# mjmyt/drone_path_planning_python

Measured on AMD Instinct MI355X. Metric: minimum-snap trajectories/sec (N drones × M segments, order 7) at 1/2/4/8 MI355X, higher is better.
Workload: dtype f64

## Files before the change

drone_path_planning_python_amd/csrc/msnap_aux.hip:

```cpp
#include <math.h>

#include <cstdlib>

#include "msnap_internal.h"
#include "msnap_energy.h"

namespace msnap {

__global__ void __launch_bounds__(256)
pack_kernel(const double *__restrict__ coef, const double *__restrict__ dur, float *__restrict__ out,
            size_t n_rows , int nc) {
  const int ncol = 1 + 4 * nc;
  const size_t total = n_rows * (size_t)ncol;
  for (size_t idx = (size_t)blockIdx.x * blockDim.x + threadIdx.x; idx < total;
       idx += (size_t)gridDim.x * blockDim.x) {
    const size_t row = idx / ncol;
    const int col = (int)(idx - row * ncol);
    const double v = (col == 0) ? dur[row] : coef[row * (size_t)(4 * nc) + (col - 1)];
    out[idx] = (float)v;
  }
}

int launch_pack(msnap_ctx *ctx, int n_drones, int n_seg, const double *coef, const double *dur, float *out) {
  const size_t rows = (size_t)n_drones * n_seg;
// ... 196 lines not shown
  const bool aligned = ((size_t)d0 * per_drone & 1) == 0;
  if (aligned) {
    for (size_t e = (size_t)tid * 2; e + 1 < words; e += (size_t)nthreads * 2)
      *reinterpret_cast<double2 *>(out + e) = *reinterpret_cast<const double2 *>(sImg + e);
    if ((words & 1) && tid == 0) out[words - 1] = sImg[words - 1];
  } else {
    for (size_t e = tid; e < words; e += nthreads) out[e] = sImg[e];
  }
  if (pos_t != nullptr) {
    const int runs = (int)per_drone;
    for (int e = tid; e < runs * nd; e += nthreads) {
      const int sk = e / nd, dl = e - sk * nd;
      pos_t[(size_t)sk * Rp + d0 + dl] = sImg[(size_t)dl * per_drone + sk];
    }
  }
  if (kbox != nullptr) {
    const int dl = tid >> 4, part = tid & 15;
    double lo[3] = {INFINITY, INFINITY, INFINITY}, hi[3] = {-INFINITY, -INFINITY, -INFINITY};
    if (dl < nd) {
      const double *img = sImg + (size_t)dl * per_drone;
      for (int sq = part; sq < S; sq += 16)
#pragma unroll
        for (int k = 0; k < 3; ++k) {
          const double v = img[(size_t)sq * 3 + k];
          if (__builtin_isfinite(v)) {
            lo[k] = v < lo[k] ? v : lo[k];
            hi[k] = v > hi[k] ? v : hi[k];
          }
        }
    }
#pragma unroll
    for (int m = 1; m < 16; m <<= 1)
#pragma unroll
      for (int k = 0; k < 3; ++k) {
        const double ol = shfl_xor_f64(lo[k], m), oh = shfl_xor_f64(hi[k], m);
        lo[k] = ol < lo[k] ? ol : lo[k];
        hi[k] = oh > hi[k] ? oh : hi[k];
      }
    if (dl < nd && part == 0) {
      double *b = kbox + (size_t)(d0 + dl) * 6;
#pragma unroll
      for (int k = 0; k < 3; ++k) {
        b[k] = lo[k];
        b[3 + k] = hi[k];
      }
      kkey[d0 + dl] = drone_sort_key(lo, hi);
    }
  }
}

__device__ __forceinline__ unsigned div_magic(unsigned d) { return d > 1 ? 0xffffffffu / d + 1u : 0u; }
__device__ __forceinline__ int div_by(int x, unsigned magic) { return magic ? (int)__umulhi((unsigned)x, magic) : x; }

template <int NC>
__global__ void __launch_bounds__(256)
sample_kernel(const double *__restrict__ coef, const double *__restrict__ dur, double dt, int N, int M, int S,
              int naxes, int DW, double *__restrict__ pos, double *__restrict__ pos_t, int Rp, double *__restrict__ kbox,
              unsigned *__restrict__ kkey) {
#pragma clang fp contract(off)
  extern __shared__ __attribute__((aligned(16))) double smem[];
  double *sB = smem;
  int *sGen = reinterpret_cast<int *>(sB + (size_t)DW * (M + 1));
  double *sImg = reinterpret_cast<double *>(sGen + ((DW + 1) & ~1));
  const int tid = threadIdx.x;
  const size_t per_drone = (size_t)S * naxes;
  const unsigned inv_piece = div_magic((unsigned)(naxes * M)), inv_axes = div_magic((unsigned)naxes);
  for (int d0 = blockIdx.x * DW; d0 < N; d0 += gridDim.x * DW) {
    const int nd = N - d0 < DW ? N - d0 : DW;
    if (tid < nd) {
      const double *dr = dur + (size_t)(d0 + tid) * M;
      double acc = 0.0;
      bool ranges = dt > 0.0;
      sB[tid * (M + 1)] = 0.0;
      for (int i = 0; i < M; ++i) {
        const double Ti = dr[i];
        ranges = ranges && (Ti >= 0.0);
        acc = acc + Ti;
        sB[tid * (M + 1) + i + 1] = acc;
      }
      sGen[tid] = ranges ? 0 : 1;
    }
    __syncthreads();
    const int items = nd * M * naxes;
    for (int it = tid; it < items; it += blockDim.x) {
      const int dl = div_by(it, inv_piece), rem = it - dl * (naxes * M);
      const int i = div_by(rem, inv_axes), a = rem - i * naxes;
      const double *cbase = coef + (size_t)(d0 + dl) * M * 4 * NC;
      double *img = sImg + (size_t)dl * per_drone;
      if (sGen[dl]) {
        if (i == 0)
          for (int sq = 0; sq < S; ++sq)
            sample_point_generic<NC>(cbase, dur + (size_t)(d0 + dl) * M, M, (double)sq * dt, a, img[(size_t)sq * naxes + a]);
        continue;
      }
      const double *crow = cbase + ((size_t)i * 4 + a) * NC;
      sample_piece<NC>(sB[dl * (M + 1) + i], sB[dl * (M + 1) + i + 1], i, M, S, dt, img, naxes, a, [&](double (&c)[NC]) {
#pragma unroll
        for (int q = 0; q < NC; q += 2) {
          const double2 v = *reinterpret_cast<const double2 *>(crow + q);
          c[q] = v.x;
          c[q + 1] = v.y;
        }
      });
    }
    __syncthreads();
    sample_image_out(sImg, tid, blockDim.x, nd, d0, per_drone, S, pos, pos_t, Rp, kbox, kkey);
    __syncthreads();
  }
}

#ifdef MSNAP_TOOLS_TIMELINE
__device__ unsigned long long g_gs_timeline[1024 * 8];
#define MSNAP_GSTL(k)                                              \
  do {                                                             \
    if (threadIdx.x == 0) s_gs_tl[(k)] = wall_clock64();           \
  } while (0)
#define MSNAP_GSTL_FLUSH()                                                                   \
  do {                                                                                       \
    lds_barrier();                                                                           \
    if (threadIdx.x < 8 && blockIdx.x < 1024) g_gs_timeline[blockIdx.x * 8 + threadIdx.x] = s_gs_tl[threadIdx.x]; \
  } while (0)
}
extern "C" int msnap_debug_read_gs_timeline(unsigned long long *out, int n_words) {
  if (hipDeviceSynchronize() != hipSuccess) return MSNAP_EHIP;
  return hipMemcpyFromSymbol(out, HIP_SYMBOL(msnap::g_gs_timeline), (size_t)n_words * 8) == hipSuccess ? MSNAP_OK : MSNAP_EHIP;
}
namespace msnap {
#else
#define MSNAP_GSTL(k) do { } while (0)
#define MSNAP_GSTL_FLUSH() do { } while (0)
#endif

typedef double v4f64s __attribute__((ext_vector_type(4)));
constexpr int kFuseKS = 3;
constexpr int kFuseTasks = 4;

template <int NC>
__global__ void __launch_bounds__(256, 2)
grid_sample_kernel(const double *__restrict__ wp, const double *__restrict__ frag, int ks_pitch,
                   const double *__restrict__ gdur, const int32_t *__restrict__ gstatus, double dt, int N, int M, int S,
                   int DW, double *__restrict__ coef, double *__restrict__ dur, int32_t *__restrict__ status,
                   double *__restrict__ pos, double *__restrict__ pos_t, int Rp, double *__restrict__ kbox,
                   unsigned *__restrict__ kkey) {
#pragma clang fp contract(off)
  extern __shared__ __attribute__((aligned(16))) double smem[];
  const int m = M + 1, ncols = M * NC, nct = (ncols + 15) >> 4, nks = (m + 3) >> 2;
  const int nrt = (DW * 4 + 15) >> 4, rows16 = nrt * 16, ntasks = nrt * nct;
  const int wpitch = m | 1, cpitch = ncols + 2;
  const int nrt_inv = nrt == 3 ? 86 : 256 >> (nrt >> 1);
  const unsigned m4_inv = (1u << 20) / (unsigned)(m * 4) + 1u;
  const unsigned inv_piece = div_magic((unsigned)(3 * M));
  double *sB = smem;
  double *sW = sB + ((m + 1) & ~1);
  double *sC = sW + (((size_t)rows16 * wpitch + 1) & ~(size_t)1);
  double *sImg = sC + (size_t)DW * 4 * cpitch;
  int *sBad = reinterpret_cast<int *>(sImg + (size_t)DW * S * 3);
  const int tid = threadIdx.x, lane = tid & (kWave - 1);
  const int wave = __builtin_amdgcn_readfirstlane(tid >> 6);
  const int col = lane & 15, kq = lane >> 4;
  const int grid_st = gstatus[0];
  const size_t per_drone = (size_t)S * 3;
#ifdef MSNAP_TOOLS_TIMELINE
  __shared__ unsigned long long s_gs_tl[8];
#endif
  MSNAP_GSTL(0);

  if (tid == 0) {
    double acc = 0.0;
    bool ranges = dt > 0.0;
    sB[0] = 0.0;
    for (int i = 0; i < M; ++i) {
      const double Ti = gdur[i];
      ranges = ranges && (Ti >= 0.0);
      acc = acc + Ti;
      sB[i + 1] = acc;
    }
    sBad[DW] = ranges ? 0 : 1;
  }
  for (int e = tid; e < rows16 * wpitch; e += blockDim.x) sW[e] = 0.0;

  for (int d0 = blockIdx.x * DW; d0 < N; d0 += gridDim.x * DW) {
    const int nd = N - d0 < DW ? N - d0 : DW;
    const int words = nd * m * 4;
    const double *wsrc = wp + (size_t)d0 * m * 4;
    const int e0 = tid, e1 = tid + 256;
    const double w0 = wsrc[e0 < words ? e0 : 0], w1 = wsrc[e1 < words ? e1 : 0];
    double bq[kFuseTasks][kFuseKS];
#pragma unroll
    for (int ti = 0; ti < kFuseTasks; ++ti) {
      const int t = wave + 4 * ti < ntasks ? wave + 4 * ti : ntasks - 1;
      const double *bsrc = frag + (size_t)((t * nrt_inv) >> 8) * ks_pitch * kWave + lane;
#pragma unroll
      for (int ks = 0; ks < kFuseKS; ++ks) bq[ti][ks] = bsrc[(ks < nks ? ks : 0) * kWave];
    }
    if (tid < DW) sBad[tid] = 0;
    lds_barrier();
    MSNAP_GSTL(1);
#pragma unroll
    for (int h = 0; h < 2; ++h) {
      const int e = h ? e1 : e0;
      const double w = h ? w1 : w0;
      if (e < words) {
        const int dl = (int)(((unsigned)e * m4_inv) >> 20), r = e - dl * (m * 4);
        sW[(size_t)(dl * 4 + (r & 3)) * wpitch + (r >> 2)] = w;
        if (!__builtin_isfinite(w)) sBad[dl] = 1;
      }
    }
    lds_barrier();
    MSNAP_GSTL(2);
    {
      double av[kFuseTasks][kFuseKS];
#pragma unroll
      for (int ti = 0; ti < kFuseTasks; ++ti) {
        const int t = wave + 4 * ti < ntasks ? wave + 4 * ti : ntasks - 1;
        const double *arow = sW + (size_t)((t - ((t * nrt_inv) >> 8) * nrt) * 16 + col) * wpitch;
#pragma unroll
        for (int ks = 0; ks < kFuseKS; ++ks) {
          const int j = 4 * ks + kq;
          const double v = arow[j < m ? j : m - 1];
          av[ti][ks] = j < m ? v : 0.0;
        }
      }
      v4f64s acc[kFuseTasks];
#pragma unroll
      for (int ti = 0; ti < kFuseTasks; ++ti) acc[ti] = v4f64s{0.0, 0.0, 0.0, 0.0};
#pragma unroll
      for (int ks = 0; ks < kFuseKS; ++ks)
        if (ks < nks) {
#pragma unroll
          for (int ti = 0; ti < kFuseTasks; ++ti)
            acc[ti] = __builtin_amdgcn_mfma_f64_16x16x4f64(av[ti][ks], bq[ti][ks], acc[ti], 0, 0, 0);
        }
#pragma unroll
      for (int ti = 0; ti < kFuseTasks; ++ti) {
        const int t = wave + 4 * ti;
        const int ct = (t * nrt_inv) >> 8, rt = t - ct * nrt;
        const int c = 16 * ct + col;
        if (t < ntasks && c < ncols) {
#pragma unroll
          for (int r = 0; r < 4; ++r) {
            const int dl = rt * 4 + r;
            if (dl < DW) sC[(size_t)(dl * 4 + kq) * cpitch + c] = acc[ti][r];
          }
        }
      }
    }
    MSNAP_GSTL(7);
    lds_barrier();
    MSNAP_GSTL(3);
    {
      const int ppd = M * 4 * NC / 2;
      for (int dl = wave; dl < nd; dl += 4) {
        const bool bad = grid_st != 0 || sBad[dl] != 0;
        double *cout = coef + (size_t)(d0 + dl) * M * 4 * NC;
        for (int e = lane; e < ppd; e += kWave) {
          const int g = 2 * e;
          const int kc = g % NC, q = g / NC;
          const int a = q & 3, seg = q >> 2;
          double2 v = *reinterpret_cast<const double2 *>(sC + (size_t)(dl * 4 + a) * cpitch + seg * NC + kc);
          if (bad) v = make_double2(__builtin_nan(""), __builtin_nan(""));
          *reinterpret_cast<double2 *>(cout + g) = v;
        }
      }
      for (int e = tid; e < nd * M; e += blockDim.x) dur[(size_t)d0 * M + e] = gdur[e % M];
      if (tid < nd) status[d0 + tid] = sBad[tid] ? MSNAP_ST_NONFINITE : grid_st;
    }
    MSNAP_GSTL(4);
    const int items = nd * M * 3;
    const bool generic = sBad[DW] != 0;
    for (int it = tid; it < items; it += blockDim.x) {
      const int dl = div_by(it, inv_piece), rem = it - dl * (3 * M);
      const int i = rem / 3, a = rem - i * 3;
      double *img = sImg + (size_t)dl * per_drone;
      const double *cbase = sC + (size_t)dl * 4 * cpitch;
      const bool bad = grid_st != 0 || sBad[dl] != 0;
      if (generic || bad) {
        if (i == 0)
          for (int sq = 0; sq < S; ++sq) {
            double x = __builtin_nan("");
            if (!bad) sample_point_generic<NC>(cbase, gdur, M, (double)sq * dt, a, x, NC, cpitch);
            img[(size_t)sq * 3 + a] = x;
          }
        continue;
      }
      const double *crow = cbase + (size_t)a * cpitch + i * NC;
      sample_piece<NC>(sB[i], sB[i + 1], i, M, S, dt, img, 3, a, [&](double (&c)[NC]) {
#pragma unroll
        for (int q = 0; q < NC; q += 2) {
          const double2 v = *reinterpret_cast<const double2 *>(crow + q);
          c[q] = v.x;
          c[q + 1] = v.y;
        }
      });
    }
    lds_barrier();
    MSNAP_GSTL(5);
    sample_image_out(sImg, tid, blockDim.x, nd, d0, per_drone, S, pos, pos_t, Rp, kbox, kkey);
    lds_barrier();
    MSNAP_GSTL(6);
  }
  MSNAP_GSTL_FLUSH();
}

__global__ void collide_key_kernel(const double *__restrict__ pos, int N, int S, double *__restrict__ box,
                                   unsigned *__restrict__ key);
constexpr int kKeyDrones = 4;

int launch_sample(msnap_ctx *ctx, int n_drones, int n_seg, const double *coef, const double *dur, double dt,
                  int n_samples, int n_axes, double *pos, double *pos_t, bool keys_form) {
  const int Rp = (n_drones + kRowBlockRows - 1) / kRowBlockRows * kRowBlockRows;
  double *kbox = keys_form ? pos_t : nullptr;
  unsigned *kkey = keys_form ? reinterpret_cast<unsigned *>(pos_t + (size_t)n_drones * 6) : nullptr;
  if (keys_form) pos_t = nullptr;
  const size_t img_per_drone = (size_t)n_samples * n_axes * sizeof(double);
  int dw = 256 / (n_seg * n_axes);
  if (dw < 1) dw = 1;
  if (dw > 16) dw = 16;
  while (dw > 1 && dw * img_per_drone > 48 * 1024) --dw;
  const size_t lds = ((size_t)dw * (n_seg + 1)) * sizeof(double) + (((size_t)dw + 1) & ~(size_t)1) * sizeof(int) +
                     dw * img_per_drone;
  if (lds <= 64 * 1024) {
    size_t blocks = ((size_t)n_drones + dw - 1) / dw;
    if (blocks > (size_t)ctx->n_cu * 64) blocks = (size_t)ctx->n_cu * 64;
    if (ctx->order == 7)
      hipLaunchKernelGGL((sample_kernel<8>), dim3((unsigned)blocks), dim3(256), lds, ctx->stream, coef, dur, dt,
                         n_drones, n_seg, n_samples, n_axes, dw, pos, pos_t, Rp, kbox, kkey);
    else
      hipLaunchKernelGGL((sample_kernel<10>), dim3((unsigned)blocks), dim3(256), lds, ctx->stream, coef, dur, dt,
                         n_drones, n_seg, n_samples, n_axes, dw, pos, pos_t, Rp, kbox, kkey);
  } else {
    const size_t total = (size_t)n_drones * n_samples;
    size_t blocks = (total + 255) / 256;
    if (blocks > (size_t)ctx->n_cu * 16) blocks = (size_t)ctx->n_cu * 16;
    if (ctx->order == 7)
      hipLaunchKernelGGL((sample_generic_kernel<8>), dim3((unsigned)blocks), dim3(256), 0, ctx->stream, coef, dur, dt,
                         n_drones, n_seg, n_samples, n_axes, pos);
    else
      hipLaunchKernelGGL((sample_generic_kernel<10>), dim3((unsigned)blocks), dim3(256), 0, ctx->stream, coef, dur, dt,
                         n_drones, n_seg, n_samples, n_axes, pos);
    if (pos_t != nullptr) {
      MSNAP_HIP(ctx, hipGetLastError());
      const int E = n_samples * 3;
      hipLaunchKernelGGL(collide_transpose_kernel, dim3(Rp / 64, (E + 31) / 32), dim3(256), 0, ctx->stream,
                         (const double *)pos, n_drones, Rp, E, pos_t, (E + 31) / 32, (int32_t *)nullptr, (size_t)0,
                         (const int32_t *)nullptr, (double *)nullptr);
    }
    if (kbox != nullptr) {
      MSNAP_HIP(ctx, hipGetLastError());
      hipLaunchKernelGGL(collide_key_kernel, dim3((n_drones + kKeyDrones - 1) / kKeyDrones), dim3(kWave * kKeyDrones), 0,
                         ctx->stream, (const double *)pos, n_drones, n_samples, kbox, kkey);
    }
  }
  MSNAP_HIP(ctx, hipGetLastError());
  return MSNAP_OK;
}

int launch_grid_sample(msnap_ctx *ctx, int n_drones, const double *wp, double dt, int n_samples, double *coef,
                       double *dur, int32_t *status, double *pos, double *pos_t, bool keys_form) {
  const int M = ctx->grid_seg, m = M + 1, nc = ctx->order + 1;
  const int ks_pitch = grid_frag_ks_pitch(ctx, M);
  const size_t img_per_drone = (size_t)n_samples * 3 * sizeof(double);
  const int ncols = M * nc, nct = (ncols + 15) / 16, nks = (m + 3) / 4;
  int dw = 256 / (M * 3);
  if (dw > 16) dw = 16;
  auto lds_of = [&](int d) -> size_t {
    const size_t rows16 = (size_t)((d * 4 + 15) / 16) * 16;
    return (size_t)(((m + 1) & ~1) + ((rows16 * (m | 1) + 1) & ~(size_t)1) + (size_t)d * 4 * (ncols + 2)) * 8 +
           d * img_per_drone + (size_t)(d + 2) * 4;
  };
  while (dw > 1 && (dw * img_per_drone > 48 * 1024 || lds_of(dw) > 64 * 1024 ||
                    ((dw * 4 + 15) / 16) * nct > 4 * kFuseTasks))
    --dw;
  const bool fused = !ctx->no_grid_sample && ks_pitch > 0 && nks <= kFuseKS && dw >= 1 && lds_of(dw) <= 64 * 1024 &&
                     ((dw * 4 + 15) / 16) * nct <= 4 * kFuseTasks && dw * (size_t)m * 4 <= 512;
  if (!fused) {
    int rc = launch_solve_grid(ctx, n_drones, wp, coef, dur, status);
    if (rc) return rc;
    return launch_sample(ctx, n_drones, M, coef, dur, dt, n_samples, 3, pos, pos_t, keys_form);
  }
  if (stream_is_capturing(ctx))
    for (DevBuf *b : {&ctx->grid_t, &ctx->grid_frag, &ctx->grid_dur, &ctx->grid_status}) b->in_graph = true;
  const int Rp = (n_drones + kRowBlockRows - 1) / kRowBlockRows * kRowBlockRows;
  double *kbox = keys_form ? pos_t : nullptr;
  unsigned *kkey = keys_form ? reinterpret_cast<unsigned *>(pos_t + (size_t)n_drones * 6) : nullptr;
  if (keys_form) pos_t = nullptr;
  size_t blocks = ((size_t)n_drones + dw - 1) / dw;
  if (blocks > (size_t)ctx->n_cu * 64) blocks = (size_t)ctx->n_cu * 64;
  note_kernel(ctx, "msnap::grid_sample_kernel<%d>", nc);
#define MSNAP_GS_LAUNCH(NCV)                                                                                            \
  hipLaunchKernelGGL((grid_sample_kernel<NCV>), dim3((unsigned)blocks), dim3(256), lds_of(dw), ctx->stream, wp,          \
                     (const double *)ctx->grid_frag.p, ks_pitch, (const double *)ctx->grid_dur.p,                         \
                     (const int32_t *)ctx->grid_status.p, dt, n_drones, M, n_samples, dw, coef, dur, status, pos, pos_t,  \
                     Rp, kbox, kkey)
  if (nc == 8) MSNAP_GS_LAUNCH(8); else MSNAP_GS_LAUNCH(10);
#undef MSNAP_GS_LAUNCH
  MSNAP_HIP(ctx, hipGetLastError());
  return MSNAP_OK;
}

template <int NC>
__device__ __forceinline__ void horner_derivs(const double *__restrict__ c, double t, double &p0, double &p1,
                                              double &p2, double &p3) {
#pragma clang fp contract(off)
  double d0[NC], d1[NC], d2[NC], d3[NC];
#pragma unroll
  for (int i = 0; i < NC; ++i) d0[i] = c[i];
#pragma unroll
  for (int i = 0; i < NC - 1; ++i) d1[i] = (double)(i + 1) * d0[i + 1];
#pragma unroll
  for (int i = 0; i < NC - 2; ++i) d2[i] = (double)(i + 1) * d1[i + 1];
#pragma unroll
  for (int i = 0; i < NC - 3; ++i) d3[i] = (double)(i + 1) * d2[i + 1];
  p0 = p1 = p2 = p3 = 0.0;
#pragma unroll
  for (int i = NC - 1; i >= 0; --i) p0 = p0 * t + d0[i];
#pragma unroll
  for (int i = NC - 2; i >= 0; --i) p1 = p1 * t + d1[i];
#pragma unroll
  for (int i = NC - 3; i >= 0; --i) p2 = p2 * t + d2[i];
#pragma unroll
  for (int i = NC - 4; i >= 0; --i) p3 = p3 * t + d3[i];
}

template <int NC>
__global__ void __launch_bounds__(256)
flat_eval_kernel(const double *__restrict__ coef, const double *__restrict__ dur, const double *__restrict__ ts,
                 int N, int M, int S, double *__restrict__ out) {
#pragma clang fp contract(off)
  __shared__ double image[256 * 13];
  const size_t total = (size_t)N * S;
  const size_t span = (size_t)gridDim.x * blockDim.x;
  const size_t trips = (total + span - 1) / span;
  for (size_t trip = 0; trip < trips; ++trip) {
    const size_t block_base = trip * span + (size_t)blockIdx.x * blockDim.x;
    const size_t idx = block_base + threadIdx.x;
    double *o = image + threadIdx.x * 13;
    if (idx < total) {
    const int d = (int)(idx / S);
    const int s = (int)(idx - (size_t)d * S);
    const double t = ts[s];
    const double *dr = dur + (size_t)d * M;
    double acc_t = 0.0;
    int seg = -1;
    for (int i = 0; i < M; ++i) {
      const double Ti = dr[i];
      if (seg < 0) {
        if (t <= acc_t + Ti) seg = i;
        else acc_t = acc_t + Ti;
      }
    }
    if (!(t >= 0.0) || seg < 0) {
#pragma unroll
      for (int q = 0; q < 13; ++q) o[q] = __builtin_nan("");
    } else {
    const double tl = t - acc_t;
    const double *c = coef + ((size_t)d * M + seg) * 4 * NC;
    double px, vx, ax, jx, py, vy, ay, jy, pz, vz, az, jz, yaw, dyaw, q2, q3;
    horner_derivs<NC>(c + 0 * NC, tl, px, vx, ax, jx);
    horner_derivs<NC>(c + 1 * NC, tl, py, vy, ay, jy);
    horner_derivs<NC>(c + 2 * NC, tl, pz, vz, az, jz);
    horner_derivs<NC>(c + 3 * NC, tl, yaw, dyaw, q2, q3);
    const double thx = ax + 0.0, thy = ay + 0.0, thz = az + 9.81;
    const double tn = sqrt(thx * thx + thy * thy + thz * thz);
    const double zbx = thx / tn, zby = thy / tn, zbz = thz / tn;
    const double xwx = cos(yaw), xwy = sin(yaw), xwz = 0.0;
    double ybx = zby * xwz - zbz * xwy, yby = zbz * xwx - zbx * xwz, ybz = zbx * xwy - zby * xwx;
    const double yn = sqrt(ybx * ybx + yby * yby + ybz * ybz);
    ybx = ybx / yn; yby = yby / yn; ybz = ybz / yn;
    const double xbx = yby * zbz - ybz * zby, xby = ybz * zbx - ybx * zbz, xbz = ybx * zby - yby * zbx;
    const double jd = jx * zbx + jy * zby + jz * zbz;
    const double hx = (jx - jd * zbx) / tn, hy = (jy - jd * zby) / tn, hz = (jz - jd * zbz) / tn;
    o[0] = px; o[1] = py; o[2] = pz;
    o[3] = vx; o[4] = vy; o[5] = vz;
    o[6] = ax; o[7] = ay; o[8] = az;
    o[9] = -(hx * ybx + hy * yby + hz * ybz);
    o[10] = hx * xbx + hy * xby + hz * xbz;
    o[11] = zbz * dyaw;
    o[12] = yaw;
    }
    }
    __syncthreads();
    const size_t ebase = block_base * 13, nelem = total * 13;
#pragma unroll
    for (int j = 0; j < 13; ++j) {
      const size_t e = (size_t)j * blockDim.x + threadIdx.x;
      if (ebase + e < nelem) out[ebase + e] = image[e];
    }
    __syncthreads();
  }
}

int launch_eval_flat(msnap_ctx *ctx, int n_drones, int n_seg, const double *coef, const double *dur,
                     int n_samples, const double *ts, double *out) {
  const size_t total = (size_t)n_drones * n_samples;
  size_t blocks = (total + 255) / 256;
  if (blocks > (size_t)ctx->n_cu * 16) blocks = (size_t)ctx->n_cu * 16;
  if (ctx->order == 7)
    hipLaunchKernelGGL((flat_eval_kernel<8>), dim3((unsigned)blocks), dim3(256), 0, ctx->stream, coef, dur, ts,
                       n_drones, n_seg, n_samples, out);
  else
    hipLaunchKernelGGL((flat_eval_kernel<10>), dim3((unsigned)blocks), dim3(256), 0, ctx->stream, coef, dur, ts,
                       n_drones, n_seg, n_samples, out);
  MSNAP_HIP(ctx, hipGetLastError());
  return MSNAP_OK;
}

template <int NC>
__global__ void __launch_bounds__(256)
snap_cost_kernel(const double *__restrict__ coef, const double *__restrict__ dur, int N, int M,
                 double *__restrict__ cost) {
  constexpr int K = NC / 2;
  const int total = N * 4;
  for (int idx = blockIdx.x * blockDim.x + threadIdx.x; idx < total; idx += gridDim.x * blockDim.x) {
    const int d = idx >> 2, a = idx & 3;
    double J = 0.0;
    for (int i = 0; i < M; ++i) {
      const double *c = coef + (((size_t)d * M + i) * 4 + a) * NC;
      const double T = dur[(size_t)d * M + i];
      double f[K];
#pragma unroll
      for (int q = 0; q < K; ++q) {
        double ff = 1.0;
#pragma unroll
        for (int r = q + 1; r <= K + q; ++r) ff *= (double)r;
        f[q] = ff * c[K + q];
      }
      double tp[2 * K];
      tp[0] = 1.0;
#pragma unroll
      for (int e = 1; e < 2 * K; ++e) tp[e] = tp[e - 1] * T;
      double acc = 0.0;
#pragma unroll
      for (int p = 0; p < K; ++p)
#pragma unroll
        for (int q = 0; q < K; ++q) acc += f[p] * f[q] * (tp[p + q + 1] / (double)(p + q + 1));
      J += acc;
    }
    cost[idx] = J;
  }
}

int launch_snap_cost(msnap_ctx *ctx, int n_drones, int n_seg, const double *coef, const double *dur, double *cost) {
  const int total = n_drones * 4;
  int blocks = (total + 255) / 256;
  if (blocks > ctx->n_cu * 8) blocks = ctx->n_cu * 8;
  if (ctx->order == 7)
    hipLaunchKernelGGL((snap_cost_kernel<8>), dim3(blocks), dim3(256), 0, ctx->stream, coef, dur, n_drones, n_seg, cost);
  else
    hipLaunchKernelGGL((snap_cost_kernel<10>), dim3(blocks), dim3(256), 0, ctx->stream, coef, dur, n_drones, n_seg, cost);
  MSNAP_HIP(ctx, hipGetLastError());
  return MSNAP_OK;
}

template <int NC>
__global__ void __launch_bounds__(256)
snap_cost_grad_kernel(const double *__restrict__ coef, size_t total, double *__restrict__ grad) {
  for (size_t idx = (size_t)blockIdx.x * blockDim.x + threadIdx.x; idx < total; idx += (size_t)gridDim.x * blockDim.x) {
    double c[NC];
#pragma unroll
    for (int j = 0; j < NC; j += 2) {
      const double2 v = *reinterpret_cast<const double2 *>(coef + idx * NC + j);
      c[j] = v.x;
      c[j + 1] = v.y;
    }
    grad[idx] = -ostrogradsky_energy<NC / 2>(c);
  }
}

int launch_snap_cost_grad(msnap_ctx *ctx, int n_drones, int n_seg, const double *coef, double *grad) {
  const size_t total = (size_t)n_drones * n_seg * 4;
  size_t blocks = (total + 255) / 256;
  if (blocks > (size_t)ctx->n_cu * 16) blocks = (size_t)ctx->n_cu * 16;
  if (ctx->order == 7)
    hipLaunchKernelGGL((snap_cost_grad_kernel<8>), dim3((unsigned)blocks), dim3(256), 0, ctx->stream, coef, total, grad);
  else
    hipLaunchKernelGGL((snap_cost_grad_kernel<10>), dim3((unsigned)blocks), dim3(256), 0, ctx->stream, coef, total, grad);
  MSNAP_HIP(ctx, hipGetLastError());
  return MSNAP_OK;
}

constexpr int kRowsPerLane = 2;
constexpr int kRowBlock = kWave * kRowsPerLane;
static_assert(kRowBlock == kRowBlockRows, "the sampler's row image uses the pairwise pass's row pitch");
constexpr int kColBlock = 8;
constexpr int kSampleChunk = 6;

struct CollideGeom {
  int R, ro, Cn, S;
  int Rp;
  int os, oe;
  int sym;
  int n_rb;
  int upw;
  int upw_tail;
  long long split;
  int sparts;
  long long total;
  long long u_lo, u_n;
  int I_lo, I_hi;
  int part;
};

__device__ __host__ __forceinline__ long long collide_ustart(const CollideGeom &g, int I) {
  return g.sym ? (long long)I * g.Cn - (long long)kRowBlock * I * (I - 1) / 2 : (long long)I * g.Cn;
}

__device__ __host__ __forceinline__ long long collide_share_begin(const CollideGeom &g, long long w) {
  const long long w1 = g.split / g.upw;
  const long long u = w <= w1 ? w * g.upw : g.split + (w - w1) * g.upw_tail;
  return g.u_lo + (u < g.u_n ? u : g.u_n);
}
__device__ __host__ __forceinline__ long long collide_share_of(const CollideGeom &g, long long u) {
  const long long ul = u - g.u_lo;
  return ul < g.split ? ul / g.upw : g.split / g.upw + (ul - g.split) / g.upw_tail;
}

typedef unsigned int u32x16 __attribute__((ext_vector_type(16)));
typedef unsigned int u32x4s __attribute__((ext_vector_type(4)));
struct ColChunk {
  u32x16 a, b;
  u32x4s c;
  __device__ __forceinline__ void fetch(const double *p) {
    asm volatile("s_load_dwordx16 %0, %3, 0x0\n\ts_load_dwordx16 %1, %3, 0x40\n\ts_load_dwordx4 %2, %3, 0x80"
                 : "=&s"(a), "=&s"(b), "=&s"(c)
                 : "s"(p));
  }
  __device__ __forceinline__ void wait(double &after) {
    asm volatile("s_waitcnt lgkmcnt(0)" : "+s"(a), "+s"(b), "+s"(c), "+v"(after));
  }
  __device__ __forceinline__ double minus(int i, double v) const {
    const unsigned long long x =
        i < 8 ? ((unsigned long long)a[2 * i + 1] << 32) | a[2 * i]
              : i < 16 ? ((unsigned long long)b[2 * (i - 8) + 1] << 32) | b[2 * (i - 8)]
                       : ((unsigned long long)c[2 * (i - 16) + 1] << 32) | c[2 * (i - 16)];
    double d;
    asm("v_add_f64 %0, %1, -%2" : "=v"(d) : "s"(x), "v"(v));
    return d;
  }
};

__device__ __forceinline__ double shfl_xor_f64(double v, int mask) {
  const int lo = __shfl_xor(__double2loint(v), mask);
  const int hi = __shfl_xor(__double2hiint(v), mask);
  return __hiloint2double(hi, lo);
}

struct RowSet {
  bool live[kRowsPerLane];
  int grow[kRowsPerLane];
  double best[kRowsPerLane];
  int bestj[kRowsPerLane];
};

struct CollideCull {
  const double *colbox;
};

__device__ __forceinline__ double box_box_lb2(const double *__restrict__ a, const double *__restrict__ b) {
#pragma clang fp contract(off)
  double gp[3];
#pragma unroll
  for (int k = 0; k < 3; ++k) {
    const double g1 = a[k] - b[3 + k], g2 = b[k] - a[3 + k];
    gp[k] = fmax(0.0, fmax(g1, g2));
  }
  return __builtin_fma(gp[2], gp[2], __builtin_fma(gp[1], gp[1], gp[0] * gp[0]));
}

template <int NC, bool CULL = false>
__device__ __forceinline__ void collide_block(const CollideGeom &g, const double *__restrict__ prowT,
                                              const double *__restrict__ pcol, int cj, int ncols, bool two_sided,
                                              RowSet &rs, int I, int h, int crow, int lane, double *sFold, int *sFoldI,
                                              double *__restrict__ cpart_d2, int32_t *__restrict__ cpart_i,
                                              const int32_t *__restrict__ oid = nullptr) {
#pragma clang fp contract(off)
  constexpr int CH = kSampleChunk, RPL = kRowsPerLane;
  const int S = g.S;
  const int stride = S * 3;
  double acc[RPL][NC];
#pragma unroll
  for (int rr = 0; rr < RPL; ++rr)
#pragma unroll
    for (int jj = 0; jj < NC; ++jj) acc[rr][jj] = INFINITY;
  const int rem = S % CH;
  const int Sw = (rem == 1 || rem == 2) ? S - rem : S;
  const int nch = (Sw + CH - 1) / CH;
  const int sc_begin = (int)((long long)nch * h / g.sparts) * CH, sc_end = (int)((long long)nch * (h + 1) / g.sparts) * CH;
  for (int sc = sc_begin; sc < sc_end; sc += CH) {
    const int s0 = (Sw - sc < CH) ? Sw - CH : sc;
    double row[RPL][CH][3];
    const double *pt = prowT + (size_t)s0 * 3 * g.Rp;
#pragma unroll
    for (int q = 0; q < CH; ++q)
#pragma unroll
      for (int k = 0; k < 3; ++k) {
        const double *pk = pt + (size_t)(3 * q + k) * g.Rp;
#pragma unroll
// ... 1740 lines not shown
```

Measured before the change: 60.61 million.

## Add streamed fused grid-solve+sample kernel for longer segment counts

```diff
diff --git a/drone_path_planning_python_amd/csrc/msnap_aux.hip b/drone_path_planning_python_amd/csrc/msnap_aux.hip
--- a/drone_path_planning_python_amd/csrc/msnap_aux.hip
+++ b/drone_path_planning_python_amd/csrc/msnap_aux.hip
@@ -522,6 +522,193 @@
   MSNAP_GSTL_FLUSH();
 }
 
+constexpr int kStreamKS = 6;
+constexpr int kStreamTiles = 4;
+constexpr int kStreamDepth = 2;
+
+template <int NC, int RT>
+__global__ void __launch_bounds__(256, 4)
+grid_stream_sample_kernel(const double *__restrict__ wp, const double *__restrict__ frag, int ks_pitch,
+                          const double *__restrict__ gdur, const int32_t *__restrict__ gstatus, double dt, int N, int M,
+                          int S, int DW, double *__restrict__ coef, double *__restrict__ dur,
+                          int32_t *__restrict__ status, double *__restrict__ pos, double *__restrict__ pos_t, int Rp,
+                          double *__restrict__ kbox, unsigned *__restrict__ kkey) {
+#pragma clang fp contract(off)
+  extern __shared__ __attribute__((aligned(16))) double smem[];
+  const int m = M + 1, ncols = M * NC, nct = (ncols + 15) >> 4, nks = (m + 3) >> 2;
+  constexpr int rows16 = RT * 16;
+  const int wpitch = m | 1, cpitch = ncols + 2;
+  const unsigned m4_inv = (1u << 20) / (unsigned)(m * 4) + 1u;
+  const int ppd = M * 4 * NC / 2;
+  const unsigned inv_piece = div_magic((unsigned)(3 * M)), inv_ppd = div_magic((unsigned)ppd);
+  const unsigned inv_m = div_magic((unsigned)M);
+  double *sB = smem;
+  double *sW = sB + ((m + 1) & ~1);
+  double *sC = sW + (((size_t)rows16 * wpitch + 1) & ~(size_t)1);
+  double *sImg = sC + (size_t)DW * 4 * cpitch;
+  int *sBad = reinterpret_cast<int *>(sImg + (size_t)DW * S * 3);
+  const int tid0 = threadIdx.x;
+  const int wave = __builtin_amdgcn_readfirstlane(tid0 >> 6);
+  const int grid_st = gstatus[0];
+  const size_t per_drone = (size_t)S * 3;
+#ifdef MSNAP_TOOLS_TIMELINE
+  __shared__ unsigned long long s_gs_tl[8];
+#endif
+  MSNAP_GSTL(0);
+
+  if (tid0 == 0) {
+    double acc = 0.0;
+    bool ranges = dt > 0.0;
+    sB[0] = 0.0;
+    for (int i = 0; i < M; ++i) {
+      const double Ti = gdur[i];
+      ranges = ranges && (Ti >= 0.0);
+      acc = acc + Ti;
+      sB[i + 1] = acc;
+    }
+    sBad[DW] = ranges ? 0 : 1;
+  }
+  for (int k = 0; k < (rows16 * wpitch + 255) >> 8; ++k) {
+    const int e = k * 256 + tid0;
+    if (e < rows16 * wpitch) sW[e] = 0.0;
+  }
+
+  for (int d0 = blockIdx.x * DW; d0 < N; d0 += gridDim.x * DW) {
+    const int nd = N - d0 < DW ? N - d0 : DW;
+    int tid = tid0;
+    asm volatile("" : "+v"(tid));
+    const int lane = tid & (kWave - 1), col = lane & 15, kq = lane >> 4;
+    const int words = nd * m * 4;
+    const double *wsrc = wp + (size_t)d0 * m * 4;
+    const int e0 = tid, e1 = tid + 256;
+    const double w0 = wsrc[e0 < words ? e0 : 0], w1 = wsrc[e1 < words ? e1 : 0];
+    double bq[kStreamTiles][kStreamKS];
+    auto load_b = [&](int ti) {
+      const int ct = wave + 4 * ti < nct ? wave + 4 * ti : nct - 1;
+      const double *bsrc = frag + (size_t)ct * ks_pitch * kWave + lane;
+#pragma unroll
+      for (int ks = 0; ks < kStreamKS; ++ks)
+        if (ks < kFuseKS + 1 || ks < nks) bq[ti][ks] = bsrc[ks * kWave];
+    };
+#pragma unroll
+    for (int ti = 0; ti < kStreamDepth && ti < kStreamTiles; ++ti) load_b(ti);
+    if (tid < DW) sBad[tid] = 0;
+    lds_barrier();
+    MSNAP_GSTL(1);
+#pragma unroll
+    for (int h = 0; h < 2; ++h) {
+      const int e = h ? e1 : e0;
+      const double w = h ? w1 : w0;
+      if (e < words) {
+        const int dl = (int)(((unsigned)e * m4_inv) >> 20), r = e - dl * (m * 4);
+        sW[(size_t)(dl * 4 + (r & 3)) * wpitch + (r >> 2)] = w;
+        if (!__builtin_isfinite(w)) sBad[dl] = 1;
+      }
+    }
+    lds_barrier();
+    MSNAP_GSTL(2);
+    {
+      double af[RT][kStreamKS];
+#pragma unroll
+      for (int rt = 0; rt < RT; ++rt) {
+        const double *arow = sW + (size_t)(rt * 16 + col) * wpitch;
+#pragma unroll
+        for (int ks = 0; ks < kStreamKS; ++ks) {
+          const int j = 4 * ks + kq;
+          const double v = arow[j < m ? j : m - 1];
+          af[rt][ks] = j < m ? v : 0.0;
+        }
+      }
+#pragma unroll
+      for (int ti = 0; ti < kStreamTiles; ++ti) {
+        if (ti + kStreamDepth < kStreamTiles) load_b(ti + kStreamDepth);
+        const int ct = wave + 4 * ti;
+        if (ct < nct) {
+          v4f64s acc[RT];
+#pragma unroll
+          for (int rt = 0; rt < RT; ++rt) acc[rt] = v4f64s{0.0, 0.0, 0.0, 0.0};
+#pragma unroll
+          for (int ks = 0; ks < kStreamKS; ++ks)
+            if (ks < kFuseKS + 1 || ks < nks) {
+#pragma unroll
+              for (int rt = 0; rt < RT; ++rt)
+                acc[rt] = __builtin_amdgcn_mfma_f64_16x16x4f64(af[rt][ks], bq[ti][ks], acc[rt], 0, 0, 0);
+            }
+          const int c = 16 * ct + col;
+          if (c < ncols) {
+#pragma unroll
+            for (int rt = 0; rt < RT; ++rt)
+#pragma unroll
+              for (int r = 0; r < 4; ++r) {
+                const int dl = rt * 4 + r;
+                if (dl < DW) sC[(size_t)(dl * 4 + kq) * cpitch + c] = acc[rt][r];
+              }
+          }
+        }
+      }
+    }
+    MSNAP_GSTL(7);
+    lds_barrier();
+    MSNAP_GSTL(3);
+    {
+      const int total = nd * ppd;
+      tid = tid0;
+      asm volatile("" : "+v"(tid));
+      double *cout = coef + (size_t)d0 * M * 4 * NC;
+      for (int k = 0; k < (total + 255) >> 8; ++k) {
+        const int e = k * 256 + tid;
+        if (e < total) {
+          const int dl = div_by(e, inv_ppd), g = 2 * (e - dl * ppd);
+          const int kc = g % NC, q = g / NC;
+          const int a = q & 3, seg = q >> 2;
+          double2 v = *reinterpret_cast<const double2 *>(sC + (size_t)(dl * 4 + a) * cpitch + seg * NC + kc);
+          if (grid_st != 0 || sBad[dl] != 0) v = make_double2(__builtin_nan(""), __builtin_nan(""));
+          *reinterpret_cast<double2 *>(cout + 2 * (size_t)e) = v;
+        }
+      }
+      if (tid < nd * M) dur[(size_t)d0 * M + tid] = gdur[tid - div_by(tid, inv_m) * M];
+      if (tid < nd) status[d0 + tid] = sBad[tid] ? MSNAP_ST_NONFINITE : grid_st;
+    }
+    MSNAP_GSTL(4);
+    const bool generic = sBad[DW] != 0;
+    tid = tid0;
+    asm volatile("" : "+v"(tid));
+    if (tid < nd * M * 3) {
+      const int dl = div_by(tid, inv_piece), rem = tid - dl * (3 * M);
+      const int i = rem / 3, a = rem - i * 3;
+      double *img = sImg + (size_t)dl * per_drone;
+      const double *cbase = sC + (size_t)dl * 4 * cpitch;
+      const bool bad = grid_st != 0 || sBad[dl] != 0;
+      if (generic || bad) {
+        if (i == 0)
+          for (int sq = 0; sq < S; ++sq) {
+            double x = __builtin_nan("");
+            if (!bad) sample_point_generic<NC>(cbase, gdur, M, (double)sq * dt, a, x, NC, cpitch);
+            img[(size_t)sq * 3 + a] = x;
+          }
+      } else {
+        const double *crow = cbase + (size_t)a * cpitch + i * NC;
+        sample_piece<NC>(sB[i], sB[i + 1], i, M, S, dt, img, 3, a, [&](double (&c)[NC]) {
+#pragma unroll
+          for (int q = 0; q < NC; q += 2) {
+            const double2 v = *reinterpret_cast<const double2 *>(crow + q);
+            c[q] = v.x;
+            c[q + 1] = v.y;
+          }
+        });
+      }
+    }
+    lds_barrier();
+    MSNAP_GSTL(5);
+    tid = tid0;
+    asm volatile("" : "+v"(tid));
+    sample_image_out(sImg, tid, blockDim.x, nd, d0, per_drone, S, pos, pos_t, Rp, kbox, kkey);
+    lds_barrier();
+    MSNAP_GSTL(6);
+  }
+  MSNAP_GSTL_FLUSH();
+}
+
 __global__ void collide_key_kernel(const double *__restrict__ pos, int N, int S, double *__restrict__ box,
                                    unsigned *__restrict__ key);
 constexpr int kKeyDrones = 4;
@@ -581,6 +768,7 @@
   const int ks_pitch = grid_frag_ks_pitch(ctx, M);
   const size_t img_per_drone = (size_t)n_samples * 3 * sizeof(double);
   const int ncols = M * nc, nct = (ncols + 15) / 16, nks = (m + 3) / 4;
+  const bool lng = nks > kFuseKS;
   int dw = 256 / (M * 3);
   if (dw > 16) dw = 16;
   auto lds_of = [&](int d) -> size_t {
@@ -589,11 +777,15 @@
            d * img_per_drone + (size_t)(d + 2) * 4;
   };
   while (dw > 1 && (dw * img_per_drone > 48 * 1024 || lds_of(dw) > 64 * 1024 ||
-                    ((dw * 4 + 15) / 16) * nct > 4 * kFuseTasks))
+                    (!lng && ((dw * 4 + 15) / 16) * nct > 4 * kFuseTasks)))
     --dw;
-  const bool fused = !ctx->no_grid_sample && ks_pitch > 0 && nks <= kFuseKS && dw >= 1 && lds_of(dw) <= 64 * 1024 &&
-                     ((dw * 4 + 15) / 16) * nct <= 4 * kFuseTasks && dw * (size_t)m * 4 <= 512;
-  if (!fused) {
+  const int nrt = (dw * 4 + 15) / 16;
+  const bool fits = !ctx->no_grid_sample && ks_pitch > 0 && dw >= 1 && lds_of(dw) <= 64 * 1024 &&
+                    dw * (size_t)m * 4 <= 512;
+  const bool fused = fits && !lng && nrt * nct <= 4 * kFuseTasks;
+  const bool stream = fits && lng && nks <= kStreamKS && nct <= 4 * kStreamTiles && nrt <= 2 &&
+                      dw * img_per_drone <= 48 * 1024;
+  if (!fused && !stream) {
     int rc = launch_solve_grid(ctx, n_drones, wp, coef, dur, status);
     if (rc) return rc;
     return launch_sample(ctx, n_drones, M, coef, dur, dt, n_samples, 3, pos, pos_t, keys_form);
@@ -606,13 +798,22 @@
   if (keys_form) pos_t = nullptr;
   size_t blocks = ((size_t)n_drones + dw - 1) / dw;
   if (blocks > (size_t)ctx->n_cu * 64) blocks = (size_t)ctx->n_cu * 64;
-  note_kernel(ctx, "msnap::grid_sample_kernel<%d>", nc);
-#define MSNAP_GS_LAUNCH(NCV)                                                                                            \
-  hipLaunchKernelGGL((grid_sample_kernel<NCV>), dim3((unsigned)blocks), dim3(256), lds_of(dw), ctx->stream, wp,          \
+#define MSNAP_GS_LAUNCH(...)                                                                                            \
+  hipLaunchKernelGGL((__VA_ARGS__), dim3((unsigned)blocks), dim3(256), lds_of(dw), ctx->stream, wp,                      \
                      (const double *)ctx->grid_frag.p, ks_pitch, (const double *)ctx->grid_dur.p,                         \
                      (const int32_t *)ctx->grid_status.p, dt, n_drones, M, n_samples, dw, coef, dur, status, pos, pos_t,  \
                      Rp, kbox, kkey)
-  if (nc == 8) MSNAP_GS_LAUNCH(8); else MSNAP_GS_LAUNCH(10);
+  if (fused) {
+    note_kernel(ctx, "msnap::grid_sample_kernel<%d>", nc);
+    if (nc == 8) MSNAP_GS_LAUNCH(grid_sample_kernel<8>); else MSNAP_GS_LAUNCH(grid_sample_kernel<10>);
+  } else {
+    note_kernel(ctx, "msnap::grid_stream_sample_kernel<%d, %d>", nc, nrt);
+    if (nc == 8) {
+      if (nrt == 1) MSNAP_GS_LAUNCH(grid_stream_sample_kernel<8, 1>); else MSNAP_GS_LAUNCH(grid_stream_sample_kernel<8, 2>);
+    } else {
+      if (nrt == 1) MSNAP_GS_LAUNCH(grid_stream_sample_kernel<10, 1>); else MSNAP_GS_LAUNCH(grid_stream_sample_kernel<10, 2>);
+    }
+  }
 #undef MSNAP_GS_LAUNCH
   MSNAP_HIP(ctx, hipGetLastError());
   return MSNAP_OK;
```

After: 59.95 million. 1.1% lower.
